# google/sbsim

Hardware: AMD Instinct MI355X
Metric: zone-updates/sec (env-steps/sec x 9 zones) at batch=64k buildings per GPU (higher is better)
Workload: dtype f64

## Files before the change

### include/sbsim_amd.h

```cpp
#ifndef SBSIM_AMD_H_
#define SBSIM_AMD_H_

#include <stddef.h>
#include <stdint.h>

#ifdef __cplusplus
extern "C" {
#endif

#define SB_ABI_VERSION 8
#define SB_NUM_ACTIONS 2
#define SB_ACTION_KEEP (-3.0e38f)
#define SB_NUM_AUX 7
#define SB_INFO_STRIDE 24

typedef enum sb_status {
  SB_OK = 0,
  SB_ERR_INVALID = -1,
  SB_ERR_NO_DEVICE = -2,
  SB_ERR_HIP = -3,
  SB_ERR_TOO_LARGE = -4,
  SB_ERR_UNSUPPORTED = -5
} sb_status;

// ... 102 lines not shown
typedef struct sb_launch_info {
  int32_t waves_per_workgroup, workgroups, lds_bytes_per_workgroup, sweep_steps;
  int64_t algorithmic_bytes_per_env_step;
  int64_t state_bytes_per_env_step;
  int32_t path;
  int32_t waves_per_building;
  int32_t kernel;
  int32_t reserved;
} sb_launch_info;

int sb_abi_version(void);
int sb_has_experimental_kernels(void);
const char *sb_last_error(void);

int sb_plan_info(const sb_plan_desc *plan, int32_t n_obs, int32_t n_buildings, sb_launch_info *out);

int sb_create(const sb_plan_desc *plan, const sb_params *params, const sb_obs_layout *obs,
              int32_t n_buildings, int32_t device, sb_handle **out);
void sb_destroy(sb_handle *h);
int sb_get_launch_info(const sb_handle *h, sb_launch_info *out);

int sb_reset(sb_handle *h, double initial_temp, const double *temps_dev, void *stream);

int sb_observe(sb_handle *h, const float aux[SB_NUM_AUX], double t_amb, const double *t_amb_dev,
               float *obs_dev, void *stream);
int sb_observe_occupancy(sb_handle *h, const float aux[SB_NUM_AUX], double t_amb, const double *t_amb_dev,
                         const float *num_occupants_dev, double occupancy_norm, float *obs_dev, void *stream);

int sb_step(sb_handle *h, const float *actions_dev, const sb_step_in *in, float *obs_dev,
            float *reward_dev, float *info_dev, void *stream);
// ... 131 lines not shown
```

### sbsim_amd/_ffi.py

```python
from __future__ import annotations

import ctypes as C
import os

_HERE = os.path.dirname(os.path.abspath(__file__))
LIB_PATH = os.environ.get("SBSIM_LIB") or os.path.join(_HERE, "libsbsim_amd.so")

SB_NUM_ACTIONS = 2
SB_ACTION_KEEP = -3.0e38
SB_NUM_AUX = 7
SB_ABI_VERSION = 8
SB_ACT_BOILER_SUPPLY_WATER_SETPOINT, SB_ACT_AHU_SUPPLY_AIR_HEATING_SETPOINT = 0, 1
SB_ACT_AHU_SUPPLY_AIR_COOLING_SETPOINT, SB_ACT_VAV_SUPPLY_AIR_DAMPER_COMMAND = 2, 3
SB_INFO_STRIDE = 24
SB_NUM_SCALARS = 16

_dp = C.POINTER(C.c_double)
_ip = C.POINTER(C.c_int32)
_fp = C.POINTER(C.c_float)


class PlanDesc(C.Structure):
  _fields_ = [("H", C.c_int32), ("W", C.c_int32), ("Z", C.c_int32), ("n_classes", C.c_int32),
              ("cell_class", C.POINTER(C.c_uint8)), ("class_coef", _dp), ("class_zone", _ip),
# ... 99 lines not shown


SB_JACOBI_COEFS = 16


class JacobiDesc(C.Structure):
  _fields_ = [("H", C.c_int32), ("W", C.c_int32), ("n_classes", C.c_int32), ("reserved", C.c_int32),
              ("cell_class", C.POINTER(C.c_uint8)), ("class_f32", _fp), ("class_diffuser", _dp), ("class_zone", _ip)]


SWEEP_KERNELS = {0: "k_sweep_lds", 1: "k_sweep_reg", 2: "k_sweep_reg (two wavefronts)", 3: "k_sweep_roll", 4: "k_sweep_two",
                 5: "k_sweep_band", 6: "k_sweep_stream", 7: "k_sweep_jacobi"}
SB_KERNEL_JACOBI = 7


EXPORTS = ("sb_abi_version", "sb_has_experimental_kernels", "sb_last_error", "sb_plan_info", "sb_create", "sb_destroy", "sb_get_launch_info",
           "sb_reset", "sb_observe", "sb_observe_occupancy", "sb_occupancy_attach", "sb_occupancy_peek", "sb_convection_attach", "sb_step", "sb_step_phases", "sb_get_temps", "sb_set_temps", "sb_get_zone_temps",
           "sb_get_scalars", "sb_get_modes", "sb_get_zone_power", "sb_debug_phase_cycles",
           "sb_floorplan_padded_shape", "sb_floorplan_preprocess", "sb_floorplan_diffusers", "sb_debug_numpy_choice", "sb_pb_reward_info", "sb_pb_reward_response",
           "sb_pb_observation_response", "sb_pb_action_response", "sb_shard_append", "sb_pb_device_info",
           "sb_pb_zone_info", "sb_pb_variable_info", "sb_record_append", "sb_tap_pre", "sb_tap_post",
           "sb_state_save", "sb_state_load", "sb_create_jacobi", "sb_tap_jacobi", "sb_set_building_params",
           "sb_set_reward_function")
STATE_ENTRIES = ("sb_state_save", "sb_state_load")
JACOBI_ENTRIES = ("sb_create_jacobi", "sb_tap_jacobi")
BUILDING_PARAM_ENTRIES = ("sb_set_building_params",)
REWARD_ENTRIES = ("sb_set_reward_function",)

_lib = None


# ... 11 lines not shown
        "(hipcc --offload-arch=gfx950).  sbsim_amd has no CPU fallback.")
  import torch
  L = C.CDLL(LIB_PATH)
  vp = C.c_void_p
  L.sb_abi_version.restype = C.c_int
  if L.sb_abi_version() != SB_ABI_VERSION:
    raise SbsimError(f"{LIB_PATH} has ABI version {L.sb_abi_version()}, this package needs {SB_ABI_VERSION}: "
                     "rebuild it (`python -c 'import __graft_entry__ as g; g.build()'`)")
  L.sb_last_error.restype = C.c_char_p
  if hasattr(L, "sb_has_experimental_kernels"):
    L.sb_has_experimental_kernels.argtypes = []
    L.sb_has_experimental_kernels.restype = C.c_int
  L.sb_create.argtypes = [C.POINTER(PlanDesc), C.POINTER(Params), C.POINTER(ObsLayout),
                          C.c_int32, C.c_int32, C.POINTER(vp)]
  L.sb_plan_info.argtypes = [C.POINTER(PlanDesc), C.c_int32, C.c_int32, C.POINTER(LaunchInfo)]
  L.sb_destroy.argtypes = [vp]
  L.sb_destroy.restype = None
  L.sb_get_launch_info.argtypes = [vp, C.POINTER(LaunchInfo)]
  L.sb_reset.argtypes = [vp, C.c_double, vp, vp]
  L.sb_observe.argtypes = [vp, C.POINTER(C.c_float), C.c_double, vp, vp, vp]
  L.sb_observe_occupancy.argtypes = [vp, C.POINTER(C.c_float), C.c_double, vp, vp, C.c_double, vp, vp]
  L.sb_occupancy_attach.argtypes = [vp, C.POINTER(OccupancyConfig)]
  L.sb_occupancy_peek.argtypes = [vp, C.c_int32, C.c_int32, vp, vp, vp]
  L.sb_convection_attach.argtypes = [vp, C.c_double, C.c_int32, C.c_uint64, C.c_int64, C.c_int32]
  L.sb_step.argtypes = [vp, vp, C.POINTER(StepIn), vp, vp, vp, vp]
  L.sb_step_phases.argtypes = [vp, vp, C.POINTER(StepIn), vp, vp, vp, vp, C.c_int32]
  for name in ("sb_get_temps", "sb_set_temps", "sb_get_zone_temps", "sb_get_scalars", "sb_get_modes",
               "sb_get_zone_power"):
    getattr(L, name).argtypes = [vp, vp, vp]
  L.sb_debug_phase_cycles.argtypes = [vp, C.POINTER(C.c_longlong)]
# ... 67 lines not shown
```

### sbsim_amd/csrc/sbsim_hip.hip

```cpp
#include <hip/hip_runtime.h>

#include <algorithm>
#include <cmath>
#include <cstdio>
#include <cstdlib>
#include <cstring>
#include <memory>
#include <string>
#include <vector>

#include "sb_host.h"

#ifndef SB_EXPERIMENTAL
namespace sb {
int launch_sweep_stream_ms(const Dev &, double *, double *, int, hipStream_t) { return (int)hipErrorNotSupported; }
int prepare_sweep_stream_ms(const Dev &, int) { return (int)hipErrorNotSupported; }
int sweep_stream_ms_sweeps() { return 1; }
int sweep_stream_ms_seam_doubles(int, int) { return 0; }
int sweep_stream_ms_xchg_doubles(int) { return 0; }
}
#endif

using namespace sb;

// ... 465 lines not shown
      for (int t = 0; t < NW; ++t) {
        const int col = t - lane;
        const int c = (R < Hs && col >= 0 && col < NS) ? cell_class(R, col) : pad;
        cw[((size_t)w * NW + t) * 64 + lane] = (uint32_t)(set_of[c] * 32) | ((uint32_t)(c * 16) << 16);
      }
      for (int s = 0; s < NS; ++s) {
        const int col = ((s - lane) % NS + NS) % NS;
        if (R < Hs && col < Ws && zone_of[(x0 + R) * W + (y0 + col)] >= 0)
          zm[((size_t)w * NS + s) * 64 + lane] = (uint16_t)zone_of[(x0 + R) * W + (y0 + col)];
      }
    }
  r.cmapS.assign((cw.size() + 1) / 2, 0);
  std::memcpy(r.cmapS.data(), cw.data(), cw.size() * sizeof(uint32_t));
  r.zmapS.assign((zm.size() + 3) / 4, 0);
  std::memcpy(r.zmapS.data(), zm.data(), zm.size() * sizeof(uint16_t));
  r.amapS.assign(1, 0);
  r.tcls.assign(1, (uint8_t)0);
  r.tcset.assign(1, (uint8_t)0);
  r.cell_state.assign(N, 0);
  int ring = 0;
  for (int x = 0; x < H; ++x)
    for (int y = 0; y < W; ++y) {
      const int R = x - x0, col = y - y0;
      if (R < 0 || R >= Hs || col < 0 || col >= Ws) { r.cell_state[x * W + y] = -(++ring); continue; }
      r.cell_state[x * W + y] = ((col + (R & 63)) % NS) * RS + R;
    }
  r.ok = true;
  return true;
}

void plan_reg(const sb_plan_desc *plan, const Trim &t, int lds_per_cu, const Knobs &k, RegPlan &r) {
  const int H = plan->H, W = plan->W, Z = plan->Z, ncls = plan->n_classes, N = H * W;
  auto coef = [&](int c, int j) { return plan->class_coef[c * 8 + j]; };
  auto cls_at = [&](int x, int y) { return (int)plan->cell_class[x * W + y]; };
  if (!t.why.empty()) { r.why = t.why; return; }
  const int x0 = t.x0, x1 = t.x1, y0 = t.y0, y1 = t.y1, Hs = t.Hs, Ws = t.Ws;
  const std::vector<int> &zone_of = t.zone_of;
  if (Hs > 64 + 2 && k.band_path && plan_band(plan, Hs, Ws, x0, y0, zone_of, k, r)) return;
  if (Hs > 64 + 2 && !k.no_two_row && plan_two(plan, Hs, Ws, x0, y0, zone_of, k, r)) return;
  if (Hs > 64 + 2 && !k.no_band && plan_band(plan, Hs, Ws, x0, y0, zone_of, k, r)) return;
// ... 643 lines not shown
extern "C" {

int sb_plan_info(const sb_plan_desc *plan, int32_t n_obs, int32_t n_buildings, sb_launch_info *out) {
  const Knobs k;
  if (!out) return fail(SB_ERR_INVALID, "sb_plan_info: null argument");
  int rc = check_plan(plan);
  if (rc != SB_OK) return rc;
  RegPlan r;
  const LdsPlan q = plan_lds(plan);
  rc = choose_kernel(plan, q, k, r);
  if (rc != SB_OK) return rc;
  fill_launch_info(plan, r, q, n_obs, capped_cus(256, k), std::max(n_buildings, 1), out);
  return SB_OK;
}

int sb_create(const sb_plan_desc *plan, const sb_params *params, const sb_obs_layout *obs,
              int32_t n_buildings, int32_t device, sb_handle **out) {
  const Knobs k;
  if (!plan || !params || !obs || !out) return fail(SB_ERR_INVALID, "sb_create: null argument");
  ActionTable acts;
  SB_CHECK(check_create_args(plan, params, obs, n_buildings, acts));
  int ndev = 0;
  if (hipGetDeviceCount(&ndev) != hipSuccess || ndev == 0)
    return fail(SB_ERR_NO_DEVICE, "sb_create: no HIP device visible (this library has no CPU path)");
  if (device < 0 || device >= ndev) return fail(SB_ERR_INVALID, "sb_create: bad device ordinal");
  SB_ON_DEVICE(device);
  hipDeviceProp_t prop;
  SB_HIP(hipGetDeviceProperties(&prop, device));

  RegPlan r;
// ... 99 lines not shown
```

### sbsim_amd/csrc/step_stream.hip

```cpp
#include "sweep_common.h"

namespace sb {
namespace {

using namespace sweep;

constexpr int kSets = 32;
#ifndef SB_STREAM_PF
#define SB_STREAM_PF 8
#endif
#ifndef SB_STREAM_ZC
#define SB_STREAM_ZC 9
#endif
#ifndef SB_STREAM_WPE
#define SB_STREAM_WPE 4
#endif
constexpr int kSpinMax = 1 << 24;
constexpr int kPF = SB_STREAM_PF;
constexpr int kZC = SB_STREAM_ZC;

extern __shared__ __attribute__((aligned(16))) double lds[];

template <int WMAX>
__global__ void __launch_bounds__(64 * WMAX)
__attribute__((amdgpu_waves_per_eu(WMAX == 2 ? 3 : SB_STREAM_WPE)))
k_sweep_stream(Dev a, double *Abuf) {
  const int lane = threadIdx.x & 63, wv = __builtin_amdgcn_readfirstlane((int)(threadIdx.x >> 6));
  const int W = (int)(blockDim.x >> 6), NS = a.NR, RS = a.RS, NSP = NS + 8;
  double *tabc = lds;
  double *tapg = lds + 4 * kSets;
  double *up = lds + a.r_seam;
  double *dn = up + (size_t)W * NSP;
  int *prog = (int *)(lds + a.r_xchg);
  double *mpart = lds + a.r_xchg + 8;
  int *misc = (int *)(lds + a.r_xchg + 24);
  double *dummy = lds + a.r_xchg + 32;
  double *zs = lds + a.r_A;
  for (int i = threadIdx.x; i < a.lds_reg_bytes / 8; i += blockDim.x) lds[i] = 0.0;
  __syncthreads();
  for (int i = threadIdx.x; i < 4 * kSets; i += blockDim.x) tabc[i] = i < 4 * a.ncset ? a.csetab[i] : 0.0;
  for (int c = threadIdx.x; c < a.ts; c += blockDim.x) tapg[2 * c] = c <= a.ncls ? a.ctab[c * 8 + 4] : 0.0;
  __syncthreads();
  if ((unsigned)(size_t)(__attribute__((address_space(3))) double *)tabc != 0u) __builtin_trap();

  const sb_params &p = a.p;
  const int row = wv * 64 + lane;
  const int NW = NS + 63;
  const unsigned *cmap_u = (const unsigned *)a.cmapS + (size_t)wv * NW * 64;
  const unsigned short *zmap_u = (const unsigned short *)a.zmapS + (size_t)wv * NS * 64;
  const unsigned lane4 = (unsigned)lane * 4u, lane2 = (unsigned)lane * 2u, row8 = (unsigned)row * 8u;
  auto cmap_at = [&](int step) { return *(const unsigned *)((const char *)(cmap_u + (size_t)step * 64) + lane4); };
  lds_vi prog_mine = (lds_vi)(unsigned)(size_t)(__attribute__((address_space(3))) int *)(prog + wv);
  lds_vi prog_prev = (lds_vi)(unsigned)(size_t)(__attribute__((address_space(3))) int *)(prog + (wv > 0 ? wv - 1 : 0));
  const double *up_prev = up + (size_t)(wv > 0 ? wv - 1 : 0) * NSP;
  const double *dn_next = dn + (size_t)(wv + 1 < W ? wv + 1 : wv) * NSP;
  const bool has_prev = wv > 0, has_next = wv + 1 < W;
  double *up_mine = up + (size_t)wv * NSP, *dn_mine = dn + (size_t)wv * NSP;
  double *const pub_dummy = dummy + (size_t)wv * 64 + lane;
  double *const pub_seam = lane == 63 ? up_mine - 63 : (lane == 0 ? dn_mine : nullptr);

  for (int b = blockIdx.x, bn = 0; b < a.B; b = bn) {
    if (threadIdx.x == 0) misc[0] = a.sweep_wgs + atomicAdd(a.next_b, 1);
    double *Eu = a.temp + (size_t)b * a.state_doubles;
    double *Au = Abuf + (size_t)blockIdx.x * a.state_doubles;
    auto E_at = [&](int slot) -> double & { return *(double *)((char *)(Eu + (size_t)slot * RS) + row8); };
    auto A_at = [&](int slot) -> double & { return *(double *)((char *)(Au + (size_t)slot * RS) + row8); };
    const double t_now = a.bld[b].t_now;
    const double ring_lo = a.scal[(size_t)b * kNScal + 16], ring_hi = a.scal[(size_t)b * kNScal + 17];
    const double ring_d = a.n_ring > 0 ? fmax(fabs(t_now - ring_lo), fabs(t_now - ring_hi)) : 0.0;
    for (int c = threadIdx.x; c < a.ts; c += blockDim.x) tapg[2 * c + 1] = a.gtabg[(size_t)b * a.ts + c];
    for (int i = threadIdx.x; i < (a.Z + 1) * kZC; i += blockDim.x) zs[i] = 0.0;
    __syncthreads();
    bn = __builtin_amdgcn_readfirstlane(*(volatile int *)misc);
    for (int s = 0; s < NS; ++s) {
      int t = s - lane;
      if (t < 0) t += NS;
      const unsigned cw = cmap_u[(size_t)(t + lane) * 64 + lane];
      const d2 pg = *(const d2 *)((const char *)tapg + (cw >> 16));
      const double v = E_at(s);
      A_at(s) = fma(pg.x, v, pg.y);
      if (lane == 0) dn_mine[s] = v;
    }
    int n_sweeps = 0, converged = 0;
    for (;;) {
      if (lane == 0) *prog_mine = 0;
      __syncthreads();
      double acc = 0.0;
      double ring_e[kPF], ring_a[kPF];
      unsigned ring_c[kPF];
      int sl = 0;
#pragma unroll
      for (int k = 0; k < kPF; ++k) {
        const int s0 = k % NS, s1 = (k + 1) % NS;
        ring_e[k] = E_at(s1);
        ring_a[k] = A_at(s0);
        ring_c[k] = cmap_at(k);
      }
      sl = kPF % NS;
      double old = E_at(0);
      double nv = 0.0;
      for (int t0 = 0; t0 < NW; t0 += kPF) {
        if (has_prev) {
          const int need = min(t0 + kPF, NS) + 63;
          while (__builtin_amdgcn_readfirstlane(*prog_prev) < need) __builtin_amdgcn_s_sleep(1);
          __builtin_amdgcn_fence(__ATOMIC_ACQUIRE, "workgroup");
        }
#pragma unroll
        for (int k = 0; k < kPF; ++k) {
          const int t = t0 + k;
          const int s = t < NS ? t : t - NS;
          const double eR = ring_e[k], Av = ring_a[k];
          const unsigned cw = ring_c[k];
          {
            const int tn = t + kPF;
            int s1 = sl + 1;
            if (s1 >= NS) s1 -= NS;
            ring_e[k] = E_at(s1);
            ring_a[k] = A_at(sl);
            ring_c[k] = cmap_at(min(tn, NW - 1));
            sl = s1;
          }
          const lds_d2 st = (lds_d2)(cw & 0xffffu);
          const d2 ud = st[0], lr = st[1];
          const int c0 = t, c63 = t - 63;
          const double rU = has_prev && c0 < NS ? up_prev[c0] : 0.0;
          const double rD = has_next && c63 >= 0 ? dn_next[c63] : 0.0;
          const double Dn = wave_shift1<0x130, true>(eR, rD);
          const double U = wave_shift1<0x138, true>(nv, rU);
          double tt = fma(ud.y, Dn, Av);
          tt = fma(lr.y, eR, tt);
          tt = fma(lr.x, nv, tt);
          const double res = fma(ud.x, U, tt);
          const int col = t - lane;
          const bool act = col >= 0 && col < NS;
          const double out = act ? res : old;
          acc = fmax(acc, fabs(out - old));
          E_at(s) = out;
          *((act && pub_seam) ? pub_seam + t : pub_dummy) = out;
          nv = act ? res : nv;
          old = eR;
        }
        __builtin_amdgcn_fence(__ATOMIC_RELEASE, "workgroup");
        if (lane == 0) *prog_mine = min(t0 + kPF, NW);
      }
      double m = wave_max(acc);
      if (lane == 0) mpart[wv] = m;
      __syncthreads();
      double md = 0.0;
      for (int w = 0; w < W; ++w) md = fmax(md, mpart[w]);
      if (n_sweeps == 0) md = fmax(md, ring_d);
      ++n_sweeps;
      converged = md <= p.conv_threshold;
      if (converged || n_sweeps >= p.iter_limit) break;
    }
    __syncthreads();
    for (int s = 0; s < NS; ++s) {
      const double v = E_at(s);
      const int z = (int)*(const unsigned short *)((const char *)(zmap_u + (size_t)s * 64) + lane2);
      __hip_atomic_fetch_add(zs + z * kZC + (lane & (kZC - 2)), v, __ATOMIC_RELAXED, __HIP_MEMORY_SCOPE_WORKGROUP);
    }
    __syncthreads();
    if (wv == 0) {
      double gacc = 0.0;
      for (int zb = 0; zb <= a.Z; zb += 64) {
        const int zz = zb + lane;
        double v = 0.0;
        if (zz <= a.Z)
          for (int k = 0; k < kZC - 1; ++k) v += zs[zz * kZC + k];
        if (zz < a.Z) a.zsum[(size_t)b * a.Z + zz] = v;
        gacc += v;
      }
      const double gsum = wave_sum(gacc);
      if (lane == 0) {
        a.gsum[b] = gsum + (double)a.n_ring * t_now;
// ... 21 lines not shown
  double *dummy = lds + a.r_xchg + 32;
  double *mpart1 = dummy + (size_t)W * 64;
  double *zs = lds + a.r_A;
  for (int i = threadIdx.x; i < a.lds_reg_bytes / 8; i += blockDim.x) lds[i] = 0.0;
  __syncthreads();
  for (int i = threadIdx.x; i < 4 * kSets; i += blockDim.x) tabc[i] = i < 4 * a.ncset ? a.csetab[i] : 0.0;
  for (int c = threadIdx.x; c < a.ts; c += blockDim.x) tapg[2 * c] = c <= a.ncls ? a.ctab[c * 8 + 4] : 0.0;
  __syncthreads();
  if ((unsigned)(size_t)(__attribute__((address_space(3))) double *)tabc != 0u) __builtin_trap();

  const sb_params &p = a.p;
  const int row = wv * 64 + lane;
  const int NW = NS + 63;
  const unsigned *cmap_u = (const unsigned *)a.cmapS + (size_t)wv * NW * 64;
  const unsigned short *zmap_u = (const unsigned short *)a.zmapS + (size_t)wv * NS * 64;
  const unsigned lane4 = (unsigned)lane * 4u, lane2 = (unsigned)lane * 2u, row8 = (unsigned)row * 8u;
  auto cmap_at = [&](int step) { return *(const unsigned *)((const char *)(cmap_u + (size_t)step * 64) + lane4); };
  lds_vi prog_mine = (lds_vi)(unsigned)(size_t)(__attribute__((address_space(3))) int *)(prog + wv);
  lds_vi prog_prev = (lds_vi)(unsigned)(size_t)(__attribute__((address_space(3))) int *)(prog + (wv > 0 ? wv - 1 : 0));
  lds_vi prog_next = (lds_vi)(unsigned)(size_t)(__attribute__((address_space(3))) int *)(prog + (wv + 1 < W ? wv + 1 : wv));
  lds_vi v_decided = (lds_vi)(unsigned)(size_t)(__attribute__((address_space(3))) int *)(misc + 2);
  lds_vi v_total = (lds_vi)(unsigned)(size_t)(__attribute__((address_space(3))) int *)(misc + 3);
  const double *up_prev = up + (size_t)(wv > 0 ? wv - 1 : 0) * NSP;
  const double *dn_next = dn + (size_t)(wv + 1 < W ? wv + 1 : wv) * NSP;
  const bool has_prev = wv > 0, has_next = wv + 1 < W;
  double *up_mine = up + (size_t)wv * NSP, *dn_mine = dn + (size_t)wv * NSP;
  double *const pub_dummy = dummy + (size_t)wv * 64 + lane;
  double *const pub_seam = lane == 63 ? up_mine - 63 : (lane == 0 ? dn_mine : nullptr);

  for (int b = blockIdx.x, bn = 0; b < a.B; b = bn) {
    if (threadIdx.x == 0) { misc[0] = a.sweep_wgs + atomicAdd(a.next_b, 1); misc[2] = 0; misc[3] = 0; misc[4] = 0; }
    if (lane == 0) *prog_mine = 0;
    double *G0 = a.temp + (size_t)b * a.state_doubles;
    double *G1 = Ebuf + (size_t)blockIdx.x * a.state_doubles;
    double *Au = Abuf + (size_t)blockIdx.x * a.state_doubles;
    auto A_at = [&](int slot) -> double & { return *(double *)((char *)(Au + (size_t)slot * RS) + row8); };
    const double t_now = a.bld[b].t_now;
    const double ring_lo = a.scal[(size_t)b * kNScal + 16], ring_hi = a.scal[(size_t)b * kNScal + 17];
    const double ring_d = a.n_ring > 0 ? fmax(fabs(t_now - ring_lo), fabs(t_now - ring_hi)) : 0.0;
    for (int c = threadIdx.x; c < a.ts; c += blockDim.x) tapg[2 * c + 1] = a.gtabg[(size_t)b * a.ts + c];
    for (int i = threadIdx.x; i < (a.Z + 1) * kZC; i += blockDim.x) zs[i] = 0.0;
    __syncthreads();
    bn = __builtin_amdgcn_readfirstlane(*(volatile int *)misc);
    for (int s = 0; s < NS; ++s) {
      int t = s - lane;
      if (t < 0) t += NS;
      const unsigned cw = cmap_u[(size_t)(t + lane) * 64 + lane];
      const d2 pg = *(const d2 *)((const char *)tapg + (cw >> 16));
      const double v = *(const double *)((const char *)(G0 + (size_t)s * RS) + row8);
      A_at(s) = fma(pg.x, v, pg.y);
      if (lane == 0) dn_mine[s] = v;
    }
    __syncthreads();
    bool stop = false;
    for (int j = 0; !stop; ++j) {
      if (j >= 2) {
        for (int spin = 0; __builtin_amdgcn_readfirstlane(*v_decided) < j - 1 && __builtin_amdgcn_readfirstlane(*v_total) == 0; ++spin) { if (spin > kSpinMax) __builtin_trap(); __builtin_amdgcn_s_sleep(1); }
      }
      if (__builtin_amdgcn_readfirstlane(*v_total) != 0) break;
      double *Gi = (j & 1) ? G1 : G0, *Go = (j & 1) ? G0 : G1;
      auto I_at = [&](int slot) -> const double & { return *(const double *)((const char *)(Gi + (size_t)slot * RS) + row8); };
      auto O_at = [&](int slot) -> double & { return *(double *)((char *)(Go + (size_t)slot * RS) + row8); };
      const int base = j * NW;
      double acc = 0.0;
      double ring_e[kPF], ring_a[kPF];
      unsigned ring_c[kPF];
      int sl = 0;
#pragma unroll
      for (int k = 0; k < kPF; ++k) {
        const int s0 = k % NS, s1 = (k + 1) % NS;
        ring_e[k] = I_at(s1);
        ring_a[k] = A_at(s0);
        ring_c[k] = cmap_at(k);
      }
      sl = kPF % NS;
      double old = I_at(0);
      double nv = 0.0;
// ... 54 lines not shown
      if (lane == 0) *prog_mine = base + NW;
      if (!has_next) {
        __builtin_amdgcn_fence(__ATOMIC_ACQUIRE, "workgroup");
        double md = 0.0;
        for (int w = 0; w < W; ++w) md = fmax(md, ((volatile double *)mp)[w]);
        if (j == 0) md = fmax(md, ring_d);
        const int conv = md <= p.conv_threshold;
        if (conv || j + 1 >= p.iter_limit) {
          if (lane == 0) { misc[4] = conv; __builtin_amdgcn_fence(__ATOMIC_RELEASE, "workgroup"); *v_total = j + 1; }
          stop = true;
        } else if (lane == 0) *v_decided = j + 1;
      }
    }
    __syncthreads();
    const int n_sweeps = misc[3], converged = misc[4];
    const double *F = (n_sweeps & 1) ? G1 : G0;
    for (int s = 0; s < NS; ++s) {
      const double v = *(const double *)((const char *)(F + (size_t)s * RS) + row8);
      if (n_sweeps & 1) *(double *)((char *)(G0 + (size_t)s * RS) + row8) = v;
      const int z = (int)*(const unsigned short *)((const char *)(zmap_u + (size_t)s * 64) + lane2);
      __hip_atomic_fetch_add(zs + z * kZC + (lane & (kZC - 2)), v, __ATOMIC_RELAXED, __HIP_MEMORY_SCOPE_WORKGROUP);
    }
    __syncthreads();
    if (wv == 0) {
      double gacc = 0.0;
      for (int zb = 0; zb <= a.Z; zb += 64) {
        const int zz = zb + lane;
        double v = 0.0;
        if (zz <= a.Z)
          for (int k = 0; k < kZC - 1; ++k) v += zs[zz * kZC + k];
        if (zz < a.Z) a.zsum[(size_t)b * a.Z + zz] = v;
        gacc += v;
      }
      const double gsum = wave_sum(gacc);
// ... 58 lines not shown
```

### sbsim_amd/csrc/step_stream_ms.hip

```cpp
#include "sweep_common.h"

namespace sb {
namespace {

using namespace sweep;

constexpr int kSets = 32;
constexpr int kPF = 8;
constexpr int kQF = 4;
constexpr int kZC = 9;
#ifndef SB_STREAM_S
#define SB_STREAM_S 4
#endif
constexpr int kS = SB_STREAM_S;

__device__ __forceinline__ unsigned used_now(unsigned v) {
  asm volatile("" : "+v"(v));
  return v;
}

extern __shared__ __attribute__((aligned(16))) double lds[];

template <int WMAX>
__global__ void __launch_bounds__(64 * WMAX) k_sweep_stream_ms(Dev a, double *Abuf, double *Ebuf) {
  const int lane = threadIdx.x & 63, wv = __builtin_amdgcn_readfirstlane((int)(threadIdx.x >> 6));
  const int W = (int)(blockDim.x >> 6), NS = a.NR, RS = a.RS, NSP = NS + 8;
  double *tabc = lds;
  double *tapg = lds + 4 * kSets;
  double *up = lds + a.r_seam;
  double *dn = up + (size_t)kS * W * NSP;
  int *prog = (int *)(lds + a.r_xchg);
  double *mpart = lds + a.r_xchg + 8;
  int *misc = (int *)(lds + a.r_xchg + 8 + kS * 16);
  double *dummy = lds + a.r_xchg + 16 + kS * 16;
  double *zs = lds + a.r_A;
  for (int i = threadIdx.x; i < a.lds_reg_bytes / 8; i += blockDim.x) lds[i] = 0.0;
  __syncthreads();
  for (int i = threadIdx.x; i < 4 * kSets; i += blockDim.x) tabc[i] = i < 4 * a.ncset ? a.csetab[i] : 0.0;
  for (int c = threadIdx.x; c < a.ts; c += blockDim.x) tapg[2 * c] = c <= a.ncls ? a.ctab[c * 8 + 4] : 0.0;
  __syncthreads();
  if ((unsigned)(size_t)(__attribute__((address_space(3))) double *)tabc != 0u) __builtin_trap();
// ... 29 lines not shown
    const double t_now = a.bld[b].t_now;
    const double ring_lo = a.scal[(size_t)b * kNScal + 16], ring_hi = a.scal[(size_t)b * kNScal + 17];
    const int prev_sweeps = a.nsw[b] & 0xffff;
    const double ring_d = a.n_ring > 0 ? fmax(fabs(t_now - ring_lo), fabs(t_now - ring_hi)) : 0.0;
    for (int c = threadIdx.x; c < a.ts; c += blockDim.x) tapg[2 * c + 1] = a.gtabg[(size_t)b * a.ts + c];
    for (int i = threadIdx.x; i < (a.Z + 1) * kZC; i += blockDim.x) zs[i] = 0.0;
    __syncthreads();
    bn = __builtin_amdgcn_readfirstlane(*(volatile int *)misc);
    {
      const unsigned *cm = cmap0 + (size_t)wv * NW * 64 + lane;
      for (int s = 0; s < NS; ++s) {
        int t = s - lane;
        if (t < 0) t += NS;
        const unsigned cw = cm[(size_t)(t + lane) * 64];
        const d2 pg = *(const d2 *)((const char *)tapg + (cw >> 16));
        Ab[(size_t)s * RS + row] = fma(pg.x, T[(size_t)s * RS + row], pg.y);
      }
    }
    int done = 0, converged = 0, Sp = min(min(max(prev_sweeps, 1), kS), p.iter_limit), redo = 0;
    int n_pass = 0, n_slots = 0;
    double md_last = 0.0, md_before = 0.0;
    const double *Ein = T;
    double *Eout = Sc;
    for (;;) {
      if (lane == 0) *prog_mine = 0;
      for (int s = lane; s < NS; s += 64) dn_mine[s] = Ein[(size_t)s * RS + 64 * wv];
      __syncthreads();
      const int NWp = NW + Sp - 1;
      ++n_pass; n_slots += Sp;
      double acc[kS], r[kS], pr[kS];
#pragma unroll
      for (int j = 0; j < kS; ++j) acc[j] = r[j] = pr[j] = 0.0;
      double ring_e[kPF], ring_a[kPF];
      unsigned ring_c[kPF];
      const unsigned *cm0 = cmap0 + (size_t)wv * NW * 64 + lane;
      auto slot_of = [&](int t) {
        t = t < 0 ? t + NS : t;
        t = t >= NS ? t - NS : t;
        return t >= NS ? t - NS : t;
      };
#pragma unroll
      for (int k = 0; k < kPF; ++k) {
        ring_e[k] = Ein[(size_t)slot_of(k + 1) * RS + row];
        ring_a[k] = Ab[(size_t)slot_of(k) * RS + row];
        ring_c[k] = cm0[(size_t)min(k, NW - 1) * 64];
      }
      double qa[kS][kQF];
      unsigned qc[kS][kQF];
#pragma unroll
      for (int j = 1; j < kS; ++j)
#pragma unroll
        for (int k = 0; k < kQF; ++k) {
          qa[j][k] = Ab[(size_t)slot_of(k - 2 * j + o64[j]) * RS + rowc[j]];
          qc[j][k] = cw_at(j, k);
        }
      double old0 = Ein[(size_t)slot_of(0) * RS + row];
      for (int t0 = 0; t0 < NWp; t0 += kPF) {
        if (has_prev) {
          const int need = min(t0 + kPF + 63, NWp);
          int spins = 0;
          while (__builtin_amdgcn_readfirstlane(*prog_prev) < need) {
            __builtin_amdgcn_s_sleep(1);
            if (++spins > (1 << 26)) __builtin_trap();
          }
          __builtin_amdgcn_fence(__ATOMIC_ACQUIRE, "workgroup");
        }
#pragma unroll
        for (int k = 0; k < kPF; ++k) {
          const int t = t0 + k;
#pragma unroll
          for (int j = kS - 1; j >= 1; --j) {
            {
              const int kq = k % kQF;
              const double Av = qa[j][kq];
              const unsigned cw = used_now(qc[j][kq]);
              {
                const int tn = t + kQF;
                qa[j][kq] = Ab[(size_t)slot_of(tn - 2 * j + o64[j]) * RS + rowc[j]];
                qc[j][kq] = cw_at(j, tn);
              }
              const int col = t - lane - j;
              const bool act = col >= 0 && col < NS && rowj[j] >= 0;
              const lds_d2 st = (lds_d2)(cw & 0xffffu);
              const d2 ud = st[0], lr = st[1];
              int c0 = t - j;
              c0 = c0 < 0 ? 0 : (c0 > NS - 1 ? NS - 1 : c0);
              const double *upj = up + ((size_t)j * W + (wv > 0 ? wv - 1 : 0)) * NSP, *upm = up + ((size_t)(j - 1) * W + (wv > 0 ? wv - 1 : 0)) * NSP;
              const double sU = upj[c0], sR = upm[c0 + 1], sO = upm[c0];
              const double R = wave_shift1<0x138, true>(r[j - 1], sR);
              const double O = wave_shift1<0x138, true>(pr[j - 1], sO);
              const double U = wave_shift1<0x138, true>(r[j], sU);
              const double D = r[j - 1], L = r[j];
              double tt = fma(ud.y, D, Av);
              tt = fma(lr.y, R, tt);
              tt = fma(lr.x, L, tt);
              const double res = fma(ud.x, U, tt);
              acc[j] = fmax(acc[j], act ? fabs(res - O) : 0.0);
              pr[j] = r[j];
              r[j] = act ? res : r[j];
              double *dst = (lane == 63 && act) ? up + ((size_t)j * W + wv) * NSP + col : pub_dummy;
              *dst = r[j];
            }
          }
          {
            const double eR = ring_e[k], Av = ring_a[k];
            const unsigned cw = used_now(ring_c[k]);
            {
              const int tn = t + kPF;
              ring_e[k] = Ein[(size_t)slot_of(tn + 1) * RS + row];
              ring_a[k] = Ab[(size_t)slot_of(tn) * RS + row];
              ring_c[k] = cm0[(size_t)min(tn, NW - 1) * 64];
            }
            const lds_d2 st = (lds_d2)(cw & 0xffffu);
            const d2 ud = st[0], lr = st[1];
            const int c0 = t, c63 = t - 63;
            const double rU = has_prev && c0 < NS ? up[(size_t)(wv > 0 ? wv - 1 : 0) * NSP + c0] : 0.0;
            const double rD = has_next && c63 >= 0 && c63 < NS ? dn_next[c63] : 0.0;
            const double Dn = wave_shift1<0x130, true>(eR, rD);
            const double U = wave_shift1<0x138, true>(r[0], rU);
            double tt = fma(ud.y, Dn, Av);
            tt = fma(lr.y, eR, tt);
            tt = fma(lr.x, r[0], tt);
            const double res = fma(ud.x, U, tt);
            const int col = t - lane;
            const bool act = col >= 0 && col < NS;
// ... 3 lines not shown
            double *dst = (lane == 63 && act) ? up + (size_t)wv * NSP + col : pub_dummy;
            *dst = r[0];
            old0 = eR;
          }
          {
            const int jl = Sp - 1;
            double v = r[0];
            int rl = row, ol = 0;
#pragma unroll
            for (int j = 1; j < kS; ++j) {
              v = jl == j ? r[j] : v;
              rl = jl == j ? rowj[j] : rl;
              ol = jl == j ? o64[j] : ol;
            }
            const int col = t - lane - jl;
            if (col < NS && rl >= 0) Eout[(size_t)slot_of(t - 2 * jl + ol) * RS + rl] = v;
          }
        }
        __builtin_amdgcn_fence(__ATOMIC_RELEASE, "workgroup");
        if (lane == 0) *prog_mine = min(t0 + kPF, NWp);
      }
#pragma unroll
      for (int j = 0; j < kS; ++j) {
        const double m = wave_max(acc[j]);
        if (lane == 0) mpart[j * 16 + wv] = m;
      }
      __syncthreads();
      double md[kS];
#pragma unroll
      for (int j = 0; j < kS; ++j) {
        md[j] = 0.0;
// ... 18 lines not shown
        if (j < Sp) { md_before = md_last; md_last = md[j]; }
      {
        const double *tmp = Eout;
        Eout = (double *)Ein;
        Ein = tmp;
      }
      int guess = 1;
      if (md_before > md_last && md_last > p.conv_threshold) {
        const double need = log(p.conv_threshold / md_last) / log(md_last / md_before);
        guess = need > (double)kS ? kS : (int)need;
      }
      Sp = min(min(max(guess, 1), kS), p.iter_limit - done);
    }
    __syncthreads();
    if (Eout != T)
      for (int s = 0; s < NS; ++s) T[(size_t)s * RS + row] = Eout[(size_t)s * RS + row];
    for (int s = 0; s < NS; ++s) {
      const double v = Eout[(size_t)s * RS + row];
      const int z = (int)zmap[(size_t)s * 64];
      __hip_atomic_fetch_add(zs + z * kZC + (lane & (kZC - 2)), v, __ATOMIC_RELAXED, __HIP_MEMORY_SCOPE_WORKGROUP);
    }
    __syncthreads();
    if (wv == 0) {
      double gacc = 0.0;
      for (int zb = 0; zb <= a.Z; zb += 64) {
        const int zz = zb + lane;
        double v = 0.0;
        if (zz <= a.Z)
          for (int k = 0; k < kZC - 1; ++k) v += zs[zz * kZC + k];
        if (zz < a.Z) a.zsum[(size_t)b * a.Z + zz] = v;
        gacc += v;
      }
      const double gsum = wave_sum(gacc);
// ... 43 lines not shown
```

Measured before the change: 302.5 million.

## Interleave slot pairs in stream-sweep state for 16-byte loads and stores

Changes the per-building state layout so that two adjacent diagonal slots of a row sit next to each other, letting the streaming sweep load and store a d2 pair per access instead of single doubles. The coefficient map is also packed into 64-bit pair words (amapS), so the prefetch ring moves half as many entries of twice the width. The other stream kernels (two-buffer and multi-sweep) are updated to the new indexing, and a new sb_plan_state_index export exposes the cell-to-state mapping to the host. The change assumes NS is even and kPF is even, raises register pressure from the d2 rings, and alters the index math in every consumer of the state layout.

```diff
diff --git a/include/sbsim_amd.h b/include/sbsim_amd.h
--- a/include/sbsim_amd.h
+++ b/include/sbsim_amd.h
@@ -140,6 +140,7 @@
 const char *sb_last_error(void);
 
 int sb_plan_info(const sb_plan_desc *plan, int32_t n_obs, int32_t n_buildings, sb_launch_info *out);
+int sb_plan_state_index(const sb_plan_desc *plan, int32_t *index, int32_t *layout);
 
 int sb_create(const sb_plan_desc *plan, const sb_params *params, const sb_obs_layout *obs,
               int32_t n_buildings, int32_t device, sb_handle **out);
diff --git a/sbsim_amd/_ffi.py b/sbsim_amd/_ffi.py
--- a/sbsim_amd/_ffi.py
+++ b/sbsim_amd/_ffi.py
@@ -137,7 +137,7 @@
 SB_KERNEL_JACOBI = 7
 
 
-EXPORTS = ("sb_abi_version", "sb_has_experimental_kernels", "sb_last_error", "sb_plan_info", "sb_create", "sb_destroy", "sb_get_launch_info",
+EXPORTS = ("sb_abi_version", "sb_has_experimental_kernels", "sb_last_error", "sb_plan_info", "sb_plan_state_index", "sb_create", "sb_destroy", "sb_get_launch_info",
            "sb_reset", "sb_observe", "sb_observe_occupancy", "sb_occupancy_attach", "sb_occupancy_peek", "sb_convection_attach", "sb_step", "sb_step_phases", "sb_get_temps", "sb_set_temps", "sb_get_zone_temps",
            "sb_get_scalars", "sb_get_modes", "sb_get_zone_power", "sb_debug_phase_cycles",
            "sb_floorplan_padded_shape", "sb_floorplan_preprocess", "sb_floorplan_diffusers", "sb_debug_numpy_choice", "sb_pb_reward_info", "sb_pb_reward_response",
@@ -179,6 +179,8 @@
   L.sb_create.argtypes = [C.POINTER(PlanDesc), C.POINTER(Params), C.POINTER(ObsLayout),
                           C.c_int32, C.c_int32, C.POINTER(vp)]
   L.sb_plan_info.argtypes = [C.POINTER(PlanDesc), C.c_int32, C.c_int32, C.POINTER(LaunchInfo)]
+  if hasattr(L, "sb_plan_state_index"):
+    L.sb_plan_state_index.argtypes = [C.POINTER(PlanDesc), C.POINTER(C.c_int32), C.POINTER(C.c_int32)]
   L.sb_destroy.argtypes = [vp]
   L.sb_destroy.restype = None
   L.sb_get_launch_info.argtypes = [vp, C.POINTER(LaunchInfo)]
diff --git a/sbsim_amd/csrc/sbsim_hip.hip b/sbsim_amd/csrc/sbsim_hip.hip
--- a/sbsim_amd/csrc/sbsim_hip.hip
+++ b/sbsim_amd/csrc/sbsim_hip.hip
@@ -503,7 +503,16 @@
   std::memcpy(r.cmapS.data(), cw.data(), cw.size() * sizeof(uint32_t));
   r.zmapS.assign((zm.size() + 3) / 4, 0);
   std::memcpy(r.zmapS.data(), zm.data(), zm.size() * sizeof(uint16_t));
-  r.amapS.assign(1, 0);
+  const int NP = (NW + 1) / 2;
+  const uint32_t pad_word = (uint32_t)(set_of[pad] * 32) | ((uint32_t)(pad * 16) << 16);
+  r.amapS.assign((size_t)NWV * NP * 64, 0);
+  for (int w = 0; w < NWV; ++w)
+    for (int P = 0; P < NP; ++P)
+      for (int lane = 0; lane < 64; ++lane) {
+        const uint32_t lo = cw[((size_t)w * NW + 2 * P) * 64 + lane];
+        const uint32_t hi = 2 * P + 1 < NW ? cw[((size_t)w * NW + 2 * P + 1) * 64 + lane] : pad_word;
+        r.amapS[((size_t)w * NP + P) * 64 + lane] = (unsigned long long)lo | ((unsigned long long)hi << 32);
+      }
   r.tcls.assign(1, (uint8_t)0);
   r.tcset.assign(1, (uint8_t)0);
   r.cell_state.assign(N, 0);
@@ -512,7 +521,8 @@
     for (int y = 0; y < W; ++y) {
       const int R = x - x0, col = y - y0;
       if (R < 0 || R >= Hs || col < 0 || col >= Ws) { r.cell_state[x * W + y] = -(++ring); continue; }
-      r.cell_state[x * W + y] = ((col + (R & 63)) % NS) * RS + R;
+      const int slot = (col + (R & 63)) % NS;
+      r.cell_state[x * W + y] = (slot / 2) * 2 * RS + R * 2 + (slot & 1);
     }
   r.ok = true;
   return true;
@@ -1186,6 +1196,27 @@
   return SB_OK;
 }
 
+int sb_plan_state_index(const sb_plan_desc *plan, int32_t *index, int32_t *layout) {
+  const Knobs k;
+  if (!index || !layout) return fail(SB_ERR_INVALID, "sb_plan_state_index: null argument");
+  int rc = check_plan(plan);
+  if (rc != SB_OK) return rc;
+  RegPlan r;
+  const LdsPlan q = plan_lds(plan);
+  rc = choose_kernel(plan, q, k, r);
+  if (rc != SB_OK) return rc;
+  const int N = plan->H * plan->W;
+  if (r.kernel == SB_KERNEL_LDS) {
+    for (int g = 0; g < N; ++g) index[g] = kPad + g;
+    layout[0] = ((N + 1) & ~1) + 2 * kPad; layout[1] = 0; layout[2] = 0;
+  } else {
+    for (int g = 0; g < N; ++g) index[g] = r.cell_state[g];
+    layout[0] = r.state_doubles; layout[1] = r.NR; layout[2] = r.RS;
+  }
+  layout[3] = (int32_t)r.kernel;
+  return SB_OK;
+}
+
 int sb_create(const sb_plan_desc *plan, const sb_params *params, const sb_obs_layout *obs,
               int32_t n_buildings, int32_t device, sb_handle **out) {
   const Knobs k;
diff --git a/sbsim_amd/csrc/step_stream.hip b/sbsim_amd/csrc/step_stream.hip
--- a/sbsim_amd/csrc/step_stream.hip
+++ b/sbsim_amd/csrc/step_stream.hip
@@ -17,6 +17,8 @@
 #endif
 constexpr int kSpinMax = 1 << 24;
 constexpr int kPF = SB_STREAM_PF;
+constexpr int kPP = kPF / 2;
+static_assert(kPF % 2 == 0 && kPF >= 2, "the prefetch depth counts whole step pairs");
 constexpr int kZC = SB_STREAM_ZC;
 
 extern __shared__ __attribute__((aligned(16))) double lds[];
@@ -46,10 +48,13 @@
   const sb_params &p = a.p;
   const int row = wv * 64 + lane;
   const int NW = NS + 63;
+  const int NH = NS >> 1, NP = (NW + 1) >> 1;
   const unsigned *cmap_u = (const unsigned *)a.cmapS + (size_t)wv * NW * 64;
   const unsigned short *zmap_u = (const unsigned short *)a.zmapS + (size_t)wv * NS * 64;
-  const unsigned lane4 = (unsigned)lane * 4u, lane2 = (unsigned)lane * 2u, row8 = (unsigned)row * 8u;
-  auto cmap_at = [&](int step) { return *(const unsigned *)((const char *)(cmap_u + (size_t)step * 64) + lane4); };
+  const unsigned long long *cmap2_u = a.amapS + (size_t)wv * NP * 64;
+  const unsigned lane8 = (unsigned)lane * 8u, lane2 = (unsigned)lane * 2u, row16 = (unsigned)row * 16u;
+  const unsigned psb = (unsigned)RS * 16u;
+  auto cmap2_at = [&](int pstep) { return *(const unsigned long long *)((const char *)(cmap2_u + (size_t)pstep * 64) + lane8); };
   lds_vi prog_mine = (lds_vi)(unsigned)(size_t)(__attribute__((address_space(3))) int *)(prog + wv);
   lds_vi prog_prev = (lds_vi)(unsigned)(size_t)(__attribute__((address_space(3))) int *)(prog + (wv > 0 ? wv - 1 : 0));
   const double *up_prev = up + (size_t)(wv > 0 ? wv - 1 : 0) * NSP;
@@ -63,8 +68,8 @@
     if (threadIdx.x == 0) misc[0] = a.sweep_wgs + atomicAdd(a.next_b, 1);
     double *Eu = a.temp + (size_t)b * a.state_doubles;
     double *Au = Abuf + (size_t)blockIdx.x * a.state_doubles;
-    auto E_at = [&](int slot) -> double & { return *(double *)((char *)(Eu + (size_t)slot * RS) + row8); };
-    auto A_at = [&](int slot) -> double & { return *(double *)((char *)(Au + (size_t)slot * RS) + row8); };
+    auto E2_at = [&](int pr) -> d2 & { return *(d2 *)((char *)Eu + ((unsigned)pr * psb + row16)); };
+    auto A2_at = [&](int pr) -> d2 & { return *(d2 *)((char *)Au + ((unsigned)pr * psb + row16)); };
     const double t_now = a.bld[b].t_now;
     const double ring_lo = a.scal[(size_t)b * kNScal + 16], ring_hi = a.scal[(size_t)b * kNScal + 17];
     const double ring_d = a.n_ring > 0 ? fmax(fabs(t_now - ring_lo), fabs(t_now - ring_hi)) : 0.0;
@@ -72,32 +77,33 @@
     for (int i = threadIdx.x; i < (a.Z + 1) * kZC; i += blockDim.x) zs[i] = 0.0;
     __syncthreads();
     bn = __builtin_amdgcn_readfirstlane(*(volatile int *)misc);
-    for (int s = 0; s < NS; ++s) {
-      int t = s - lane;
-      if (t < 0) t += NS;
-      const unsigned cw = cmap_u[(size_t)(t + lane) * 64 + lane];
-      const d2 pg = *(const d2 *)((const char *)tapg + (cw >> 16));
-      const double v = E_at(s);
-      A_at(s) = fma(pg.x, v, pg.y);
-      if (lane == 0) dn_mine[s] = v;
+    for (int pr = 0; pr < NH; ++pr) {
+      const int s = 2 * pr;
+      const int st0 = s < lane ? s + NS : s, st1 = s + 1 < lane ? s + 1 + NS : s + 1;
+      const unsigned cw0 = cmap_u[(size_t)st0 * 64 + lane], cw1 = cmap_u[(size_t)st1 * 64 + lane];
+      const d2 pg0 = *(const d2 *)((const char *)tapg + (cw0 >> 16)), pg1 = *(const d2 *)((const char *)tapg + (cw1 >> 16));
+      const d2 v = E2_at(pr);
+      d2 av;
+      av.x = fma(pg0.x, v.x, pg0.y); av.y = fma(pg1.x, v.y, pg1.y);
+      A2_at(pr) = av;
+      if (lane == 0) { dn_mine[s] = v.x; dn_mine[s + 1] = v.y; }
     }
     int n_sweeps = 0, converged = 0;
     for (;;) {
       if (lane == 0) *prog_mine = 0;
       __syncthreads();
       double acc = 0.0;
-      double ring_e[kPF], ring_a[kPF];
-      unsigned ring_c[kPF];
-      int sl = 0;
+      d2 ring_e[kPP], ring_a[kPP];
+      unsigned long long ring_c[kPP];
+      int pl = 0;
 #pragma unroll
-      for (int k = 0; k < kPF; ++k) {
-        const int s0 = k % NS, s1 = (k + 1) % NS;
-        ring_e[k] = E_at(s1);
-        ring_a[k] = A_at(s0);
-        ring_c[k] = cmap_at(k);
-      }
-      sl = kPF % NS;
-      double old = E_at(0);
+      for (int k = 0; k < kPP; ++k) {
+        ring_e[k] = E2_at((k + 1) % NH);
+        ring_a[k] = A2_at(k % NH);
+        ring_c[k] = cmap2_at(k);
+      }
+      pl = kPP % NH;
+      d2 cur = E2_at(0);
       double nv = 0.0;
       for (int t0 = 0; t0 < NW; t0 += kPF) {
         if (has_prev) {
@@ -106,39 +112,44 @@
           __builtin_amdgcn_fence(__ATOMIC_ACQUIRE, "workgroup");
         }
 #pragma unroll
-        for (int k = 0; k < kPF; ++k) {
-          const int t = t0 + k;
+        for (int k = 0; k < kPP; ++k) {
+          const int t = t0 + 2 * k;
           const int s = t < NS ? t : t - NS;
-          const double eR = ring_e[k], Av = ring_a[k];
-          const unsigned cw = ring_c[k];
+          const d2 nxt = ring_e[k], Av2 = ring_a[k];
+          const unsigned long long cw2 = ring_c[k];
           {
-            const int tn = t + kPF;
-            int s1 = sl + 1;
-            if (s1 >= NS) s1 -= NS;
-            ring_e[k] = E_at(s1);
-            ring_a[k] = A_at(sl);
-            ring_c[k] = cmap_at(min(tn, NW - 1));
-            sl = s1;
+            int p1 = pl + 1;
+            if (p1 >= NH) p1 -= NH;
+            ring_e[k] = E2_at(p1);
+            ring_a[k] = A2_at(pl);
+            ring_c[k] = cmap2_at(min((t >> 1) + kPP, NP - 1));
+            pl = p1;
           }
-          const lds_d2 st = (lds_d2)(cw & 0xffffu);
-          const d2 ud = st[0], lr = st[1];
-          const int c0 = t, c63 = t - 63;
-          const double rU = has_prev && c0 < NS ? up_prev[c0] : 0.0;
-          const double rD = has_next && c63 >= 0 ? dn_next[c63] : 0.0;
-          const double Dn = wave_shift1<0x130, true>(eR, rD);
-          const double U = wave_shift1<0x138, true>(nv, rU);
-          double tt = fma(ud.y, Dn, Av);
-          tt = fma(lr.y, eR, tt);
-          tt = fma(lr.x, nv, tt);
-          const double res = fma(ud.x, U, tt);
-          const int col = t - lane;
-          const bool act = col >= 0 && col < NS;
-          const double out = act ? res : old;
-          acc = fmax(acc, fabs(out - old));
-          E_at(s) = out;
-          *((act && pub_seam) ? pub_seam + t : pub_dummy) = out;
-          nv = act ? res : nv;
-          old = eR;
+          auto step = [&](int t, double old, double eR, double Av, unsigned cw) {
+            const lds_d2 st = (lds_d2)(cw & 0xffffu);
+            const d2 ud = st[0], lr = st[1];
+            const int c0 = t, c63 = t - 63;
+            const double rU = has_prev && c0 < NS ? up_prev[c0] : 0.0;
+            const double rD = has_next && c63 >= 0 ? dn_next[c63] : 0.0;
+            const double Dn = wave_shift1<0x130, true>(eR, rD);
+            const double U = wave_shift1<0x138, true>(nv, rU);
+            double tt = fma(ud.y, Dn, Av);
+            tt = fma(lr.y, eR, tt);
+            tt = fma(lr.x, nv, tt);
+            const double res = fma(ud.x, U, tt);
+            const int col = t - lane;
+            const bool act = col >= 0 && col < NS;
+            const double out = act ? res : old;
+            acc = fmax(acc, fabs(out - old));
+            *((act && pub_seam) ? pub_seam + t : pub_dummy) = out;
+            nv = act ? res : nv;
+            return out;
+          };
+          d2 o2;
+          o2.x = step(t, cur.x, cur.y, Av2.x, (unsigned)cw2);
+          o2.y = step(t + 1, cur.y, nxt.x, Av2.y, (unsigned)(cw2 >> 32));
+          E2_at(s >> 1) = o2;
+          cur = nxt;
         }
         __builtin_amdgcn_fence(__ATOMIC_RELEASE, "workgroup");
         if (lane == 0) *prog_mine = min(t0 + kPF, NW);
@@ -154,10 +165,12 @@
       if (converged || n_sweeps >= p.iter_limit) break;
     }
     __syncthreads();
-    for (int s = 0; s < NS; ++s) {
-      const double v = E_at(s);
-      const int z = (int)*(const unsigned short *)((const char *)(zmap_u + (size_t)s * 64) + lane2);
-      __hip_atomic_fetch_add(zs + z * kZC + (lane & (kZC - 2)), v, __ATOMIC_RELAXED, __HIP_MEMORY_SCOPE_WORKGROUP);
+    for (int pr = 0; pr < NH; ++pr) {
+      const d2 v = E2_at(pr);
+      const int z0 = (int)*(const unsigned short *)((const char *)(zmap_u + (size_t)(2 * pr) * 64) + lane2);
+      const int z1 = (int)*(const unsigned short *)((const char *)(zmap_u + (size_t)(2 * pr + 1) * 64) + lane2);
+      __hip_atomic_fetch_add(zs + z0 * kZC + (lane & (kZC - 2)), v.x, __ATOMIC_RELAXED, __HIP_MEMORY_SCOPE_WORKGROUP);
+      __hip_atomic_fetch_add(zs + z1 * kZC + (lane & (kZC - 2)), v.y, __ATOMIC_RELAXED, __HIP_MEMORY_SCOPE_WORKGROUP);
     }
     __syncthreads();
     if (wv == 0) {
@@ -209,7 +222,8 @@
   const int NW = NS + 63;
   const unsigned *cmap_u = (const unsigned *)a.cmapS + (size_t)wv * NW * 64;
   const unsigned short *zmap_u = (const unsigned short *)a.zmapS + (size_t)wv * NS * 64;
-  const unsigned lane4 = (unsigned)lane * 4u, lane2 = (unsigned)lane * 2u, row8 = (unsigned)row * 8u;
+  const unsigned lane4 = (unsigned)lane * 4u, lane2 = (unsigned)lane * 2u, row16 = (unsigned)row * 16u;
+  auto at = [&](double *G, int slot) -> double & { return *(double *)((char *)(G + (size_t)(slot >> 1) * 2 * RS + (slot & 1)) + row16); };
   auto cmap_at = [&](int step) { return *(const unsigned *)((const char *)(cmap_u + (size_t)step * 64) + lane4); };
   lds_vi prog_mine = (lds_vi)(unsigned)(size_t)(__attribute__((address_space(3))) int *)(prog + wv);
   lds_vi prog_prev = (lds_vi)(unsigned)(size_t)(__attribute__((address_space(3))) int *)(prog + (wv > 0 ? wv - 1 : 0));
@@ -229,7 +243,7 @@
     double *G0 = a.temp + (size_t)b * a.state_doubles;
     double *G1 = Ebuf + (size_t)blockIdx.x * a.state_doubles;
     double *Au = Abuf + (size_t)blockIdx.x * a.state_doubles;
-    auto A_at = [&](int slot) -> double & { return *(double *)((char *)(Au + (size_t)slot * RS) + row8); };
+    auto A_at = [&](int slot) -> double & { return at(Au, slot); };
     const double t_now = a.bld[b].t_now;
     const double ring_lo = a.scal[(size_t)b * kNScal + 16], ring_hi = a.scal[(size_t)b * kNScal + 17];
     const double ring_d = a.n_ring > 0 ? fmax(fabs(t_now - ring_lo), fabs(t_now - ring_hi)) : 0.0;
@@ -242,7 +256,7 @@
       if (t < 0) t += NS;
       const unsigned cw = cmap_u[(size_t)(t + lane) * 64 + lane];
       const d2 pg = *(const d2 *)((const char *)tapg + (cw >> 16));
-      const double v = *(const double *)((const char *)(G0 + (size_t)s * RS) + row8);
+      const double v = at(G0, s);
       A_at(s) = fma(pg.x, v, pg.y);
       if (lane == 0) dn_mine[s] = v;
     }
@@ -254,8 +268,8 @@
       }
       if (__builtin_amdgcn_readfirstlane(*v_total) != 0) break;
       double *Gi = (j & 1) ? G1 : G0, *Go = (j & 1) ? G0 : G1;
-      auto I_at = [&](int slot) -> const double & { return *(const double *)((const char *)(Gi + (size_t)slot * RS) + row8); };
-      auto O_at = [&](int slot) -> double & { return *(double *)((char *)(Go + (size_t)slot * RS) + row8); };
+      auto I_at = [&](int slot) -> const double & { return at(Gi, slot); };
+      auto O_at = [&](int slot) -> double & { return at(Go, slot); };
       const int base = j * NW;
       double acc = 0.0;
       double ring_e[kPF], ring_a[kPF];
@@ -340,10 +354,10 @@
     }
     __syncthreads();
     const int n_sweeps = misc[3], converged = misc[4];
-    const double *F = (n_sweeps & 1) ? G1 : G0;
+    double *F = (n_sweeps & 1) ? G1 : G0;
     for (int s = 0; s < NS; ++s) {
-      const double v = *(const double *)((const char *)(F + (size_t)s * RS) + row8);
-      if (n_sweeps & 1) *(double *)((char *)(G0 + (size_t)s * RS) + row8) = v;
+      const double v = at(F, s);
+      if (n_sweeps & 1) at(G0, s) = v;
       const int z = (int)*(const unsigned short *)((const char *)(zmap_u + (size_t)s * 64) + lane2);
       __hip_atomic_fetch_add(zs + z * kZC + (lane & (kZC - 2)), v, __ATOMIC_RELAXED, __HIP_MEMORY_SCOPE_WORKGROUP);
     }
diff --git a/sbsim_amd/csrc/step_stream_ms.hip b/sbsim_amd/csrc/step_stream_ms.hip
--- a/sbsim_amd/csrc/step_stream_ms.hip
+++ b/sbsim_amd/csrc/step_stream_ms.hip
@@ -25,6 +25,7 @@
 __global__ void __launch_bounds__(64 * WMAX) k_sweep_stream_ms(Dev a, double *Abuf, double *Ebuf) {
   const int lane = threadIdx.x & 63, wv = __builtin_amdgcn_readfirstlane((int)(threadIdx.x >> 6));
   const int W = (int)(blockDim.x >> 6), NS = a.NR, RS = a.RS, NSP = NS + 8;
+  auto sidx = [&](int s, int r) -> size_t { return ((size_t)(s >> 1) * RS + r) * 2 + (s & 1); };
   double *tabc = lds;
   double *tapg = lds + 4 * kSets;
   double *up = lds + a.r_seam;
@@ -84,7 +85,7 @@
         if (t < 0) t += NS;
         const unsigned cw = cm[(size_t)(t + lane) * 64];
         const d2 pg = *(const d2 *)((const char *)tapg + (cw >> 16));
-        Ab[(size_t)s * RS + row] = fma(pg.x, T[(size_t)s * RS + row], pg.y);
+        Ab[sidx(s, row)] = fma(pg.x, T[sidx(s, row)], pg.y);
       }
     }
     int done = 0, converged = 0, Sp = min(min(max(prev_sweeps, 1), kS), p.iter_limit), redo = 0;
@@ -94,7 +95,7 @@
     double *Eout = Sc;
     for (;;) {
       if (lane == 0) *prog_mine = 0;
-      for (int s = lane; s < NS; s += 64) dn_mine[s] = Ein[(size_t)s * RS + 64 * wv];
+      for (int s = lane; s < NS; s += 64) dn_mine[s] = Ein[sidx(s, 64 * wv)];
       __syncthreads();
       const int NWp = NW + Sp - 1;
       ++n_pass; n_slots += Sp;
@@ -111,8 +112,8 @@
       };
 #pragma unroll
       for (int k = 0; k < kPF; ++k) {
-        ring_e[k] = Ein[(size_t)slot_of(k + 1) * RS + row];
-        ring_a[k] = Ab[(size_t)slot_of(k) * RS + row];
+        ring_e[k] = Ein[sidx(slot_of(k + 1), row)];
+        ring_a[k] = Ab[sidx(slot_of(k), row)];
         ring_c[k] = cm0[(size_t)min(k, NW - 1) * 64];
       }
       double qa[kS][kQF];
@@ -121,10 +122,10 @@
       for (int j = 1; j < kS; ++j)
 #pragma unroll
         for (int k = 0; k < kQF; ++k) {
-          qa[j][k] = Ab[(size_t)slot_of(k - 2 * j + o64[j]) * RS + rowc[j]];
+          qa[j][k] = Ab[sidx(slot_of(k - 2 * j + o64[j]), rowc[j])];
           qc[j][k] = cw_at(j, k);
         }
-      double old0 = Ein[(size_t)slot_of(0) * RS + row];
+      double old0 = Ein[sidx(slot_of(0), row)];
       for (int t0 = 0; t0 < NWp; t0 += kPF) {
         if (has_prev) {
           const int need = min(t0 + kPF + 63, NWp);
@@ -146,7 +147,7 @@
               const unsigned cw = used_now(qc[j][kq]);
               {
                 const int tn = t + kQF;
-                qa[j][kq] = Ab[(size_t)slot_of(tn - 2 * j + o64[j]) * RS + rowc[j]];
+                qa[j][kq] = Ab[sidx(slot_of(tn - 2 * j + o64[j]), rowc[j])];
                 qc[j][kq] = cw_at(j, tn);
               }
               const int col = t - lane - j;
@@ -177,8 +178,8 @@
             const unsigned cw = used_now(ring_c[k]);
             {
               const int tn = t + kPF;
-              ring_e[k] = Ein[(size_t)slot_of(tn + 1) * RS + row];
-              ring_a[k] = Ab[(size_t)slot_of(tn) * RS + row];
+              ring_e[k] = Ein[sidx(slot_of(tn + 1), row)];
+              ring_a[k] = Ab[sidx(slot_of(tn), row)];
               ring_c[k] = cm0[(size_t)min(tn, NW - 1) * 64];
             }
             const lds_d2 st = (lds_d2)(cw & 0xffffu);
@@ -212,7 +213,7 @@
               ol = jl == j ? o64[j] : ol;
             }
             const int col = t - lane - jl;
-            if (col < NS && rl >= 0) Eout[(size_t)slot_of(t - 2 * jl + ol) * RS + rl] = v;
+            if (col < NS && rl >= 0) Eout[sidx(slot_of(t - 2 * jl + ol), rl)] = v;
           }
         }
         __builtin_amdgcn_fence(__ATOMIC_RELEASE, "workgroup");
@@ -261,9 +262,9 @@
     }
     __syncthreads();
     if (Eout != T)
-      for (int s = 0; s < NS; ++s) T[(size_t)s * RS + row] = Eout[(size_t)s * RS + row];
+      for (int s = 0; s < NS; ++s) T[sidx(s, row)] = Eout[sidx(s, row)];
     for (int s = 0; s < NS; ++s) {
-      const double v = Eout[(size_t)s * RS + row];
+      const double v = Eout[sidx(s, row)];
       const int z = (int)zmap[(size_t)s * 64];
       __hip_atomic_fetch_add(zs + z * kZC + (lane & (kZC - 2)), v, __ATOMIC_RELAXED, __HIP_MEMORY_SCOPE_WORKGROUP);
     }
```

Result: no change. 302.6 million (median of 2 runs) (+0.0%).
